# Emieeel/auto_oo

Measured on AMD Instinct MI355X. Metric: OO-VQE energy+grad evals/sec (formaldimine CAS(4e,3o)/cc-pVDZ); 2e-transform fp64 TFLOP/s vs roofline, higher is better.
Workload: dtype f64; 1 GPU; configs[1] shape: N=43 AOs, n_occ=6, CAS(4e,3o), UCCD n_theta=4, n_kappa=327; one step = one batched call evaluating energy + full gradient of all 256 geometries of the rank (256 synthetic geometries in the job, geometry g on rank g mod n_gpus); value = evaluations/s; in-order calls on one stream; geometries_per_rank=256, batched_calls=1332, calls=in order, parallelism=geometry-sharded x1, one all_gather at the end, dist_world_size=1, devices_visible=1, device_of_rank0=0

## Files before the change

auto_oo_amd/csrc/api.hip:

```cpp
#include "common.h"
#include <stdarg.h>
#include <map>
#include <mutex>
#include <tuple>
#include <utility>
#include <vector>

static thread_local char g_err[512] = "";

void oovqe_set_error(const char* fmt, ...)
{
    va_list ap;
    va_start(ap, fmt);
    vsnprintf(g_err, sizeof(g_err), fmt, ap);
    va_end(ap);
}

extern "C" int oovqe_version(void) { return 100; }

extern "C" const char* oovqe_last_error(void) { return g_err; }

extern "C" int oovqe_device_count(void)
{
    int n = 0;
    hipError_t e = hipGetDeviceCount(&n);
    if (e != hipSuccess) {
        oovqe_set_error("hipGetDeviceCount: %s", hipGetErrorString(e));
        return -1;
    }
    return n;
}

int oovqe_ensure_dynamic_lds(const void* kernel, size_t bytes)
{
    static std::mutex mu;
    static std::map<std::pair<const void*, int>, size_t> done;
    int dev = 0;
    if (hipGetDevice(&dev) != hipSuccess) dev = 0;
    std::lock_guard<std::mutex> lock(mu);
    size_t& have = done[std::make_pair(kernel, dev)];
    if (bytes <= have) return 0;
    hipError_t e = hipFuncSetAttribute(kernel, hipFuncAttributeMaxDynamicSharedMemorySize, (int)bytes);
    if (e != hipSuccess) {
        oovqe_set_error("hipFuncSetAttribute(MaxDynamicSharedMemorySize = %zu): %s", bytes, hipGetErrorString(e));
        return OOVQE_ERR_HIP;
    }
    have = bytes;
    return 0;
}

int oovqe_blocks_per_cu(const void* kernel, int threads, size_t lds_bytes)
{
    static std::mutex mu;
    static std::map<std::tuple<const void*, int, int, size_t>, int> known;
    int dev = 0;
    if (hipGetDevice(&dev) != hipSuccess) dev = 0;
    std::lock_guard<std::mutex> lock(mu);
    int& occ = known[std::make_tuple(kernel, dev, threads, lds_bytes)];
    if (occ > 0) return occ;
    int nb = 0;
    OOVQE_CHECK_HIP(hipOccupancyMaxActiveBlocksPerMultiprocessor(&nb, kernel, threads, lds_bytes), "oovqe_blocks_per_cu");
    return occ = nb < 1 ? 1 : nb;
}

int oovqe_cu_count()
{
    static int n_cu[16];
    static std::mutex mu;
    int dev = 0;
    if (hipGetDevice(&dev) != hipSuccess || dev < 0 || dev >= 16) return 256;
    std::lock_guard<std::mutex> lock(mu);
    if (!n_cu[dev]) {
        hipDeviceProp_t prop;
        n_cu[dev] = hipGetDeviceProperties(&prop, dev) == hipSuccess && prop.multiProcessorCount > 0 ? prop.multiProcessorCount : 256;
    }
    return n_cu[dev];
}

static int g_opts[OOVQE_OPT_COUNT] = {0};
static const char* const g_opt_names[OOVQE_OPT_COUNT] = {
    "gm_two_per_cu", "gm_one_per_cu", "fused_chunks", "tri_plain_w", "cas_unfused",
    "sym_no_rs", "sym_mirror", "sym_simple", "sym_two_step", "no_ride", "k1_no_pair", "k1_force_wide", "gm_plain_grid",
    "newton_one_wg", "sector_unfused", "hess_vk_pass", "hess_own_stage1", "panel_rows",
    "k1_force_nt", "newton_no_chol", "sector_lambda_w", "sector_rdm_r3", "panel_no_w",
    "stage1_free_run", "one_stream", "tail_split"};
static_assert(sizeof(g_opt_names) / sizeof(g_opt_names[0]) == OOVQE_OPT_COUNT, "option name table out of step with oovqe_option_t");

int oovqe_opt(int id) { return (id >= 0 && id < OOVQE_OPT_COUNT) ? g_opts[id] : 0; }

static char g_stage1[160] = "";
void oovqe_note_stage1(const char* fmt, ...)
{
    va_list ap;
    va_start(ap, fmt);
    vsnprintf(g_stage1, sizeof(g_stage1), fmt, ap);
    va_end(ap);
}
extern "C" const char* oovqe_last_stage1_kernel(void) { return g_stage1; }

extern "C" int oovqe_debug_set_option(const char* name, int value)
{
    for (int i = 0; name && i < OOVQE_OPT_COUNT; ++i)
        if (strcmp(name, g_opt_names[i]) == 0) { g_opts[i] = value; return 0; }
    oovqe_set_error("oovqe_debug_set_option: unknown option '%s'", name ? name : "(null)");
    return OOVQE_ERR_ARG;
}

extern "C" int oovqe_debug_get_option(const char* name)
{
    for (int i = 0; name && i < OOVQE_OPT_COUNT; ++i)
        if (strcmp(name, g_opt_names[i]) == 0) return g_opts[i];
    return -1;
}

namespace {
struct Internals {
    hipEvent_t ev[64] = {};
    hipStream_t st[1] = {nullptr};
    unsigned next = 0;
    bool tried = false, streams_tried = false;
};
Internals g_int[16];
std::mutex g_int_mu;

Internals* internals()
{
    int dev = 0;
    if (hipGetDevice(&dev) != hipSuccess || dev < 0 || dev >= 16) return nullptr;
    Internals& I = g_int[dev];
    if (!I.tried) {
        I.tried = true;
        for (int i = 0; i < 64; ++i)
            if (hipEventCreateWithFlags(&I.ev[i], hipEventDisableTiming) != hipSuccess) I.ev[i] = nullptr;
    }
    return &I;
}
}

hipEvent_t oovqe_internal_event()
{
    std::lock_guard<std::mutex> lock(g_int_mu);
    Internals* I = internals();
    return I ? I->ev[I->next++ & 63] : nullptr;
}

hipStream_t oovqe_internal_stream(int k)
{
    if (oovqe_opt(OOVQE_OPT_ONE_STREAM) != 0 || k != 0) return nullptr;
    std::lock_guard<std::mutex> lock(g_int_mu);
    Internals* I = internals();
    if (!I) return nullptr;
    if (!I->streams_tried) {
        I->streams_tried = true;
        if (hipStreamCreateWithFlags(&I->st[0], hipStreamNonBlocking) != hipSuccess) I->st[0] = nullptr;
    }
    return I->st[k];
}

static hipStream_t g_s1_stream[16];
static hipEvent_t g_s1_event[16];
static bool g_s1_seen[16];
static int g_s1_multi[16];

int oovqe_stage1_enter(hipStream_t st)
{
    int dev = 0;
    if (hipGetDevice(&dev) != hipSuccess || dev < 0 || dev >= 16) return 0;
    if (oovqe_opt(OOVQE_OPT_STAGE1_FREE_RUN) != 0) return 0;
// ... 123 lines not shown
```

auto_oo_amd/csrc/cas.hip:

```cpp
#include "plan.h"
#include "circuit_small.h"
#include <type_traits>
#include <stdlib.h>

namespace {

constexpr int HALF_WAVES = 8;
constexpr int TRI_REG_R = 3;
constexpr int tiles_depth(int zt) { return zt == 3 ? 4 : 8; }
constexpr int stream_depth(int zt) { return zt == 3 ? 2 : 3; }
constexpr int AUX_PLAIN = 0, AUX_NT = 2;

constexpr int SYM_FULL = 0, SYM_MIRROR = 1, SYM_PACKED = 2;
__device__ __forceinline__ void tri_decode(long t, int N, int& p, int& q)
{
    const double b = 2.0 * N + 1.0;
    int pp = (int)((b - sqrt(b * b - 8.0 * (double)t)) * 0.5);
    pp = pp < 0 ? 0 : (pp > N - 1 ? N - 1 : pp);
    while (pp > 0 && (long)pp * (2 * N - pp + 1) / 2 > t) --pp;
    while (pp < N - 1 && (long)(pp + 1) * (2 * N - pp) / 2 <= t) ++pp;
    p = pp;
    q = pp + (int)(t - (long)pp * (2 * N - pp + 1) / 2);
}

// ... 2333 lines not shown
        int rr[4], cc[4], kk[4];
#pragma unroll
        for (int u = 0; u < 4; ++u) {
            const long idx = base + u * 512 + tid;
            const bool ok = idx < (long)nrdm * n_kappa;
            const long ii = ok ? idx : 0;
            kk[u] = (int)(ii / n_kappa);
            const int t = (int)(ii - (long)kk[u] * n_kappa);
            rr[u] = kap_row[t];
            cc[u] = kap_col[t];
        }
        double frc[4], fcr[4];
#pragma unroll
        for (int u = 0; u < 4; ++u) {
            const double* F = Fcol + (size_t)kk[u] * M * N;
            const int r = rr[u], c = cc[u];
            frc[u] = F[(size_t)(r < M ? r : 0) * N + c] * (r < M ? 1.0 : 0.0);
            fcr[u] = F[(size_t)(c < M ? c : 0) * N + r] * (c < M ? 1.0 : 0.0);
        }
#pragma unroll
        for (int u = 0; u < 4; ++u) {
            const long idx = base + u * 512 + tid;
            if (idx < (long)nrdm * n_kappa) gvec[idx] = 2.0 * (frc[u] - fcr[u]);
        }
    }
    if (fock)
        for (int idx = tid; idx < N * N; idx += 512) {
            const int m = idx / N;
            fock[idx] = m < M ? Fcol[idx] : 0.0;
        }
    if (gmat)
        for (int idx = tid; idx < N * N; idx += 512) {
            const int m = idx / N, n = idx - m * N;
            const double fmn = m < M ? Fcol[(size_t)m * N + n] : 0.0;
            const double fnm = n < M ? Fcol[(size_t)n * N + m] : 0.0;
            gmat[idx] = 2.0 * (fmn - fnm);
        }
    if (tid < nrdm) {
        const int k = tid;
        double acc = 0.0;
        for (int n = 0; n < M; ++n) acc += Epart[(size_t)k * N + n];
        if (k == 0) {
            double core = nuc;
            for (int n = 0; n < M; ++n) core += Cpart[n];
            c0[0] = core;
            E[0] = core + acc;
        } else if (dE) {
            dE[k - 1] = acc;
        }
    }
}

constexpr int TAIL_THREADS = 512;

__host__ __device__ inline bool tail_needed(int x, int y, int z, int no)
{
    const int lo = y < z ? y : z, hi = y < z ? z : y;
    if (lo >= no) return true;
    if (hi < no) return lo == hi || x == lo || x == hi;
    return x >= no || x == lo;
}
__host__ __device__ inline int tail_pitch(int NC) { return 16 * (((NC + 15) / 16) | 1); }

#ifdef OOVQE_TAIL_PROBE
constexpr int TAIL_PROBE_WGS = 512, TAIL_PROBE_MARKS = 32;
__device__ long long g_tail_probe[TAIL_PROBE_WGS][TAIL_PROBE_MARKS];
#define TAIL_MARK(i)                                                                              \
    do {                                                                                          \
        __syncthreads();                                                                          \
        if (threadIdx.x == 0 && blockIdx.x < TAIL_PROBE_WGS && (i) < TAIL_PROBE_MARKS)            \
            g_tail_probe[blockIdx.x][i] = wall_clock64();                                         \
    } while (0)
#else
#define TAIL_MARK(i) do {} while (0)
#endif

template <int KS>
__global__ __launch_bounds__(TAIL_THREADS, 2)
void cas_tail_kernel(const double* __restrict__ J, const double* __restrict__ C, const double* __restrict__ Wpre,
                     const double* __restrict__ gamma, const double* __restrict__ Gamma, int nrdm, int N, int no,
                     int na, int NC, double nuc, const double* __restrict__ nuc_arr,
                     const int32_t* __restrict__ kap_row, const int32_t* __restrict__ kap_col, int n_kappa,
                     double* __restrict__ c0, double* __restrict__ E, double* __restrict__ gvec,
                     double* __restrict__ dE, double* __restrict__ c1, double* __restrict__ c2, size_t out_stride)
{
    extern __shared__ double lds[];
    constexpr int NW = TAIL_THREADS / 64;
    constexpr int PW = (4 * KS + NW - 1) / NW;
    constexpr int GR = 2, NG = (PW + GR - 1) / GR;
    constexpr int NTN = (4 * KS + 15) / 16;
    const int M = no + na, M2 = M * M, M3 = M2 * M;
    const int na2 = na * na, na3 = na2 * na, na4 = na2 * na2;
    const int ncol = M * (M + 1) / 2, nty = (ncol + 15) / 16;
    const long tri = (long)N * (N + 1) / 2;
    const int by = blockIdx.x;
    const int tid = threadIdx.x, lane = tid & 63;
    const int wave = __builtin_amdgcn_readfirstlane(tid >> 6);
    const int lq = lane >> 4, lr = lane & 15;
    {
        const size_t gi = by;
        J += gi * nty * tri * 16;
        C += gi * (size_t)N * N;
        Wpre += gi * (size_t)N * N;
        gamma += gi * (size_t)nrdm * na2;
        Gamma += gi * (size_t)nrdm * na4;
        c0 += gi * out_stride;
        E += gi * out_stride;
        gvec += gi * out_stride;
        if (dE) dE += gi * out_stride;
        c1 += gi * out_stride;
        c2 += gi * out_stride;
        if (nuc_arr) nuc = nuc_arr[gi];
    }
    const int LDG = tail_pitch(NC), nct = (NC + 15) / 16;
    double* Gc = lds;
    double* Cl = Gc + (size_t)4 * KS * LDG;
    double* hn = Cl + (size_t)N * M;
    double* FIn = hn + (size_t)N * M;
    double* gml = FIn + (size_t)N * M;
    double* Gml = gml + (size_t)nrdm * na2;
    double* Cp = Gml + (size_t)nrdm * na4;
    int* tab = reinterpret_cast<int*>(Cp + N);
    int* wcnt = tab + M3;
    int* krow = wcnt + NW;
    int* kcol = krow + n_kappa;
    double* scr = Cp + N + (M3 + NW + 2 * n_kappa + 1) / 2;
    int* tabp = reinterpret_cast<int*>(scr + (size_t)N * N);

    typedef unsigned v2u __attribute__((ext_vector_type(2)));
    constexpr bool COLQ_REGS = KS < 12;
    int colq[KS];
#pragma unroll
    for (int ks = 0; ks < KS; ++ks) {
        const int q = 4 * ks + lq < N ? 4 * ks + lq : N - 1;
        colq[ks] = ((q * (2 * N - q + 1) / 2 - q) * 16 + lr) * (int)sizeof(double);
    }
    const int lin0 = (lq * 16 + lr) * (int)sizeof(double);
    auto load_group = [&](double (&bf)[GR][KS], int ty, int g) {
#pragma unroll
        for (int r = 0; r < GR; ++r) {
            const int i = g * GR + r;
            if (i >= PW) continue;
            int wv = wave;
#if defined(__HIP_DEVICE_COMPILE__)
            asm volatile("" : "+s"(wv));
#endif
            const int p = wv + NW * i;
            int lqo = lq;
#if defined(__HIP_DEVICE_COMPILE__)
            asm volatile("" : "+v"(lqo));
#endif
            const __amdgpu_buffer_rsrc_t jsrd = __builtin_amdgcn_make_buffer_rsrc(
                const_cast<double*>(J + (size_t)(ty < nty ? ty : 0) * tri * 16), 0,
                p < N && ty < nty ? (int)(tri * 16 * sizeof(double)) : 0, 0x00020000);
            const int colp = p * 16 * (int)sizeof(double);
            const int rowp = (p * (2 * N - p + 1) / 2 - p) * 16 * (int)sizeof(double) + lin0;
#pragma unroll
            for (int ks = 0; ks < KS; ++ks) {
                const int q = 4 * ks + lqo;
                const int cq = COLQ_REGS ? colq[ks] : (q * (2 * N - 1 - q) / 2 * 16 + lr) * (int)sizeof(double);
                const int off = lq < p - 4 * ks ? cq + colp : rowp + ks * 64 * (int)sizeof(double);
                const v2u v = __builtin_amdgcn_raw_buffer_load_b64(jsrd, (unsigned)off, 0, 0);
                bf[r][ks] = __builtin_bit_cast(double, v);
            }
        }
    };
    auto mfma_group = [&](const double (&af)[KS], const double (&bf)[GR][KS], const int (&tj)[4], int g) {
#pragma unroll
        for (int r = 0; r < GR; ++r) {
            const int i = g * GR + r;
            if (i >= PW) continue;
            int wv = wave;
#if defined(__HIP_DEVICE_COMPILE__)
            asm volatile("" : "+s"(wv));
#endif
            const int p = wv + NW * i;
            if (p >= 4 * KS) continue;
            d4 acc = d4{0.0, 0.0, 0.0, 0.0};
            if (p < N) {
#pragma unroll
                for (int ks = 0; ks < KS; ++ks) acc = mfma_f64(af[ks], bf[r][ks], acc);
            }
            double* row = Gc + p * LDG;
#pragma unroll
            for (int j = 0; j < 4; ++j)
                if (tj[j] >= 0) row[tj[j]] = acc[j];
        }
    };
    double bs[2][GR][KS];
    TAIL_MARK(0);
#pragma unroll
    for (int s0 = 0; s0 < 2; ++s0) load_group(bs[s0], s0 / NG, s0 % NG);

    for (int idx = tid; idx < N * M; idx += TAIL_THREADS) {
        const int q = idx / M, x = idx - q * M;
        Cl[idx] = C[(size_t)q * N + x];
    }
    for (int idx = tid; idx < N * N; idx += TAIL_THREADS) scr[idx] = Wpre[idx];
    for (int idx = tid; idx < nrdm * na2; idx += TAIL_THREADS) gml[idx] = gamma[idx];
    for (int idx = tid; idx < nrdm * na4; idx += TAIL_THREADS) Gml[idx] = Gamma[idx];
    for (int idx = tid; idx < n_kappa; idx += TAIL_THREADS) {
        krow[idx] = kap_row[idx];
        kcol[idx] = kap_col[idx];
    }
    for (int idx = tid; idx < 4 * KS * (LDG - NC); idx += TAIL_THREADS) {
        const int p = idx / (LDG - NC);
        Gc[p * LDG + NC + (idx - p * (LDG - NC))] = 0.0;
    }
    TAIL_MARK(1);
    {
        const int total = M * ncol;
        int base = 0;
        for (int i0 = 0; i0 < total; i0 += TAIL_THREADS) {
            const int i = i0 + tid;
            int x = 0, y = 0, z = 0;
            bool need = false;
            if (i < total) {
                x = i / ncol;
                tri_decode(i - x * ncol, M, y, z);
                need = tail_needed(x, y, z, no);
            }
            const unsigned long long mask = __ballot(need);
            const int below = __popcll(mask & ((1ull << lane) - 1ull));
            if (lane == 0) wcnt[wave] = __popcll(mask);
            __syncthreads();
            int pre = base, all = 0;
            for (int w = 0; w < NW; ++w) {
                const int c = wcnt[w];
                if (w < wave) pre += c;
                all += c;
            }
            if (i < total) {
                const int v = need ? pre + below : -1;
                tab[(x * M + y) * M + z] = v;
                tab[(x * M + z) * M + y] = v;
                tabp[i] = v;
            }
            __syncthreads();
            base += all;
        }
    }
    TAIL_MARK(2);
    for (int idx = tid; idx < N * M; idx += TAIL_THREADS) {
        const int n = idx / M, x = idx - n * M;
        double acc = 0.0;
        for (int q = 0; q < N; ++q) acc += scr[(size_t)n * N + q] * Cl[q * M + x];
        hn[idx] = acc;
    }
    __syncthreads();
    TAIL_MARK(3);

    {
        double af[KS];
#pragma unroll
        for (int ks = 0; ks < KS; ++ks) {
            const int q = 4 * ks + lq;
            const double c = Cl[(q < N ? q : N - 1) * M + (lr < M ? lr : 0)];
            af[ks] = (q < N && lr < M) ? c : 0.0;
        }
        auto tail_tile = [&](auto par, int ty) {
            constexpr int P = decltype(par)::value;
            const int yz = 16 * ty + lr;
            int tj[4];
#pragma unroll
            for (int j = 0; j < 4; ++j) {
                const int x = lq + 4 * j;
                tj[j] = (x < M && yz < ncol) ? tabp[x * ncol + yz] : -1;
            }
#pragma unroll
            for (int g = 0; g < NG; ++g) {
                mfma_group(af, bs[(P + g) & 1], tj, g);
                __builtin_amdgcn_sched_barrier(0);
                load_group(bs[(P + g) & 1], ty + (g + 2) / NG, (g + 2) % NG);
                __builtin_amdgcn_sched_barrier(0);
            }
        };
        for (int ty = 0; ty < nty; ty += 2) {
            tail_tile(std::integral_constant<int, 0>{}, ty);
            if (ty + 1 < nty) tail_tile(std::integral_constant<int, NG & 1>{}, ty + 1);
        }
    }

    {
        const __amdgpu_buffer_rsrc_t csrd = __builtin_amdgcn_make_buffer_rsrc(
            const_cast<double*>(C), 0, (int)((size_t)N * N * sizeof(double)), 0x00020000);
        double cfa[NTN][KS];
#pragma unroll
        for (int nt = 0; nt < NTN; ++nt)
#pragma unroll
            for (int ks = 0; ks < KS; ++ks) {
                const int pp = 4 * ks + lq, n = 16 * nt + lr;
                const v2u v = __builtin_amdgcn_raw_buffer_load_b64(
                    csrd, (pp < N && n < N) ? (unsigned)((pp * N + n) * (int)sizeof(double)) : 0x7fffffffu, 0, 0);
                cfa[nt][ks] = __builtin_bit_cast(double, v);
            }
        __syncthreads();
        TAIL_MARK(4);
        const int ntn = (N + 15) / 16;
        for (int ct = wave; ct < nct; ct += NW) {
            double* col = Gc + (16 * ct + lr);
            double tf[KS];
#pragma unroll
            for (int ks = 0; ks < KS; ++ks) tf[ks] = col[(4 * ks + lq) * LDG];
#pragma unroll
            for (int nt = 0; nt < NTN; ++nt) {
                if (nt >= ntn) continue;
                d4 acc = d4{0.0, 0.0, 0.0, 0.0};
#pragma unroll
                for (int ks = 0; ks < KS; ++ks) acc = mfma_f64(cfa[nt][ks], tf[ks], acc);
#pragma unroll
                for (int j = 0; j < 4; ++j) {
                    const int n = 16 * nt + lq + 4 * j;
                    if (n < N) col[n * LDG] = acc[j];
                }
            }
        }
        __syncthreads();
        TAIL_MARK(5);
    }

#define TAIL_G(n, a, b, c) Gc[(n) * LDG + tab[((a) * M + (b)) * M + (c)]]
    for (int idx = tid; idx < N * M; idx += TAIL_THREADS) {
        const int n = idx / M, x = idx - n * M;
        double fi = hn[idx];
        for (int i = 0; i < no; ++i) fi += 2.0 * TAIL_G(n, x, i, i) - TAIL_G(n, i, i, x);
        FIn[idx] = fi;
    }
    TAIL_MARK(6);
    double* Fl = scr;
    double* El = Fl + (size_t)nrdm * M * N;
    double* Ga = El + (size_t)nrdm * N;
    double* Dc = Ga + (size_t)N * na3;
    for (int idx = tid; idx < N * na3; idx += TAIL_THREADS) {
        const int n = idx / na3, r = idx - n * na3;
        const int w = r / na2, x = (r / na) % na, y = r % na;
        Ga[idx] = TAIL_G(n, no + w, no + x, no + y);
    }
    for (int idx = tid; idx < N * no * na2; idx += TAIL_THREADS) {
        const int n = idx / (no * na2), r = idx - n * (no * na2);
        const int m = r / na2, v = (r / na) % na, w = r % na;
        const int V = no + v, W = no + w;
        Dc[idx] = TAIL_G(n, m, V, W) - 0.5 * TAIL_G(n, W, V, m);
    }
    __syncthreads();
    TAIL_MARK(7);
    for (int n = tid; n < N; n += TAIL_THREADS) Cp[n] = n < no ? hn[n * M + n] + FIn[n * M + n] : 0.0;
    for (int idx = tid; idx < na * (na + na3); idx += TAIL_THREADS) {
        const int pl = idx / (na + na3), r0 = idx - pl * (na + na3);
        const int n = no + pl;
        if (r0 < na) {
            c1[pl * na + r0] = FIn[n * M + no + r0];
        } else {
            int t = r0 - na;
            const int i3 = t;
            const int s = t % na; t /= na;
            const int r = t % na; t /= na;
            const int q = t;
            c2[(size_t)pl * na3 + i3] = 0.5 * TAIL_G(n, no + q, no + r, no + s);
        }
    }
    TAIL_MARK(8);
    const int ncore = N * nrdm * no;
    for (int idx = tid; idx < N * nrdm * M; idx += TAIL_THREADS) {
        int n, k, m;
        if (idx < ncore) {
            n = idx / (nrdm * no);
            const int r0 = idx - n * (nrdm * no);
            k = r0 / no;
            m = r0 - k * no;
        } else {
            const int j = idx - ncore;
            n = j / (nrdm * na);
            const int r0 = j - n * (nrdm * na);
            k = r0 / na;
            m = no + r0 - k * na;
        }
        const double* FIv = FIn + (size_t)n * M;
        const double* gam = gml + (size_t)k * na2;
        double val;
        if (m < no) {
            const double* Dm = Dc + ((size_t)n * no + m) * na2;
            double fa = 0.0;
            for (int v = 0; v < na; ++v)
                for (int w = 0; w < na; ++w) fa += gam[v * na + w] * Dm[v * na + w];
            val = 2.0 * ((k == 0 ? FIv[m] : 0.0) + fa);
        } else {
            const int v = m - no;
            const double* Gv = Gml + (size_t)k * na4 + (size_t)v * na3;
            double acc = 0.0;
            for (int w = 0; w < na; ++w) acc += FIv[no + w] * gam[v * na + w];
            for (int w = 0; w < na; ++w)
                for (int x = 0; x < na; ++x)
                    for (int y = 0; y < na; ++y)
                        acc += Gv[(w * na + x) * na + y] * Ga[(size_t)n * na3 + (w * na + x) * na + y];
            val = acc;
        }
        Fl[((size_t)k * M + m) * N + n] = val;
    }
    TAIL_MARK(9);
    for (int idx = tid; idx < N * nrdm; idx += TAIL_THREADS) {
        const int n = idx / nrdm, k = idx - n * nrdm;
        double acc = 0.0;
        if (n >= no && n < M) {
            const int p = n - no;
            const double* FIv = FIn + (size_t)n * M;
            const double* gam = gml + (size_t)k * na2 + (size_t)p * na;
            const double* Gpq = Gml + (size_t)k * na4 + (size_t)p * na3;
            for (int q = 0; q < na; ++q) acc += FIv[no + q] * gam[q];
            for (int q = 0; q < na; ++q)
                for (int r = 0; r < na; ++r)
                    for (int s2 = 0; s2 < na; ++s2)
                        acc += 0.5 * Ga[(size_t)n * na3 + (q * na + r) * na + s2] * Gpq[(q * na + r) * na + s2];
        }
        El[(size_t)k * N + n] = acc;
    }
#undef TAIL_G
    __syncthreads();
    TAIL_MARK(10);

    for (int idx = tid; idx < nrdm * n_kappa; idx += TAIL_THREADS) {
        const int k = idx / n_kappa, t = idx - k * n_kappa;
        const int r = krow[t], c = kcol[t];
        const double* F = Fl + (size_t)k * M * N;
        const double frc = F[(size_t)(r < M ? r : 0) * N + c] * (r < M ? 1.0 : 0.0);
        const double fcr = F[(size_t)(c < M ? c : 0) * N + r] * (c < M ? 1.0 : 0.0);
        gvec[idx] = 2.0 * (frc - fcr);
    }
    if (tid < nrdm) {
        const int k = tid;
        double acc = 0.0;
        for (int n = 0; n < M; ++n) acc += El[(size_t)k * N + n];
        if (k == 0) {
            double core = nuc;
            for (int n = 0; n < M; ++n) core += Cp[n];
            c0[0] = core;
            E[0] = core + acc;
        } else if (dE) {
            dE[k - 1] = acc;
        }
    }
    TAIL_MARK(11);
}

}

#ifdef OOVQE_TAIL_PROBE
extern "C" int oovqe_tail_probe_read(long long* out, int n)
{
    const size_t bytes = sizeof(long long) * (size_t)(n < TAIL_PROBE_WGS * TAIL_PROBE_MARKS ? n : TAIL_PROBE_WGS * TAIL_PROBE_MARKS);
    return hipMemcpyFromSymbol(out, HIP_SYMBOL(g_tail_probe), bytes) == hipSuccess ? 0 : 1;
}
#endif

#define OOVQE_STAGE1_DISPATCH(v, LAUNCH, ...)                                                     \
    switch ((v).kch) {                                                                            \
    case 4: LAUNCH(4, 1, 2, ##__VA_ARGS__); break;                                                \
    case 8: LAUNCH(8, 2, 5, ##__VA_ARGS__); break;                                                \
    case 11: LAUNCH(11, 3, 8, ##__VA_ARGS__); break;                                              \
    default: LAUNCH(12, 3, 10, ##__VA_ARGS__); break;                                             \
    }
#define OOVQE_KS_DISPATCH(v, LAUNCH)                                                              \
    switch ((v).ks) {                                                                             \
    case 4: LAUNCH(4); break;                                                                     \
    case 8: LAUNCH(8); break;                                                                     \
    default: LAUNCH(12); break;                                                                   \
    }

static int stage1_variant(int N, Stage1Variant* v)
{
    static const Stage1Variant rows[] = {{4, 1, 2, 4}, {8, 2, 5, 8}, {11, 3, 8, 12}, {12, 3, 10, 12}};
    for (const Stage1Variant& r : rows)
        if (N >= 1 && (N + 3) / 4 <= r.kch) {
            *v = r;
            return 0;
        }
    oovqe_set_error("cas_eval: no stage-1 kernel variant for N=%d", N);
    return OOVQE_ERR_ARG;
}

static size_t half_lds_bytes(int N, int M)
{
    const int ZT = (M + 15) / 16, nrb = (N + 15) / 16, LDM = 16 * (ZT | 1);
    return (((size_t)nrb * 16 * LDM + 511) / 512) * 512 * sizeof(double);
}
static size_t half_lds_bytes_rs(int N, int M) { return half_lds_bytes(N, M) + (size_t)HALF_WAVES * 16 * 17 * sizeof(double); }

static int stage1_half(int N, int M, int sym, bool rs, bool tiles, Stage1* s)
{
    memset(s, 0, sizeof(*s));
    OOVQE_REQUIRE(N >= 1 && M >= 1 && M <= N, "cas_half_transform: bad N=%d M=%d", N, M);
    const int ZT = (M + 15) / 16, nrb = (N + 15) / 16, ksteps = (N + 3) / 4;
    OOVQE_REQUIRE(ZT <= 3, "cas_half_transform: n_occ+ncas = %d > 48 not supported", M);
    OOVQE_REQUIRE(half_lds_bytes(N, M) <= 160 * 1024, "cas_half_transform: N=%d M=%d needs %zu B of LDS", N, M,
                  half_lds_bytes(N, M));
    s->zt = ZT;
    s->sym = sym;
    if (nrb <= 3) {
        s->kernel = S1_HALF;
// ... 191 lines not shown
    oovqe_profile_mark_stop(st);
    OOVQE_CHECK_LAUNCH("cas_eval/sym_q_contract");
    return 0;
}

static int sym_gm_batched(const double* J, const double* C, double* Gm, int N, int M, int batch,
                          hipStream_t st, const oovqe_circuit_job_t* cj, bool packed)
{
    OOVQE_REQUIRE(M >= 1 && M <= 16 && N >= 1 && N <= 48, "sym_gm: N=%d M=%d", N, M);
    Stage1Variant v;
    if (int rc = stage1_variant(N, &v)) return rc;
    size_t lds_bytes = (size_t)4 * v.ks * (M * 16 + 8) * sizeof(double);
    if (cj && cj->lds_bytes > lds_bytes) lds_bytes = cj->lds_bytes;
    const unsigned nty = (unsigned)(((packed ? M * (M + 1) / 2 : M * M) + 15) / 16);
    oovqe_circuit_job_t job;
    memset(&job, 0, sizeof(job));
    if (cj) job = *cj;
    const unsigned nx = nty + (cj ? 1 : 0);
    const bool xcd_grid = oovqe_xcd_grid(batch, oovqe_opt(OOVQE_OPT_GM_PLAIN_GRID) != 0);
    const dim3 grid = xcd_grid ? dim3(nx * (unsigned)((batch + 7) / 8 * 8)) : dim3(nx, batch);
#define OOVQE_LAUNCH_GM2(KS_, WPE_)                                                               \
    do {                                                                                          \
        if (int rc_ = oovqe_ensure_dynamic_lds((const void*)sym_gm_kernel<KS_, WPE_>, lds_bytes)) return rc_; \
        hipLaunchKernelGGL((sym_gm_kernel<KS_, WPE_>), grid, dim3(SMALL_THREADS), lds_bytes, st,  \
                           J, C, Gm, N, M, packed ? 1 : 0, job, cj ? 1 : 0, batch);               \
    } while (0)
    const bool multi_round = ((long)nx * batch > (long)oovqe_cu_count() || oovqe_opt(OOVQE_OPT_GM_TWO_PER_CU)) &&
                             2 * lds_bytes <= 160 * 1024 && oovqe_opt(OOVQE_OPT_GM_ONE_PER_CU) == 0;
#define OOVQE_LAUNCH_GM(KS_)                                                                      \
    do {                                                                                          \
        if (multi_round) OOVQE_LAUNCH_GM2(KS_, 4);                                                \
        else OOVQE_LAUNCH_GM2(KS_, 2);                                                            \
    } while (0)
    oovqe_profile_mark_start_l(st, LABEL_P_TO_N);
    OOVQE_KS_DISPATCH(v, OOVQE_LAUNCH_GM)
    oovqe_profile_mark_stop(st);
#undef OOVQE_LAUNCH_GM
#undef OOVQE_LAUNCH_GM2
    OOVQE_CHECK_LAUNCH("cas_eval/sym_gm");
    return 0;
}

static int tail_depth(int N, const Stage1Variant& v) { return N >= 41 && N <= 44 ? 11 : v.ks; }
#define OOVQE_TAIL_DISPATCH(ks, LAUNCH)                                                           \
    switch (ks) {                                                                                 \
    case 4: LAUNCH(4); break;                                                                     \
    case 8: LAUNCH(8); break;                                                                     \
    case 11: LAUNCH(11); break;                                                                   \
    default: LAUNCH(12); break;                                                                   \
    }

static size_t tail_lds_bytes(int N, int no, int na, int nrdm, int n_kappa, int* NC)
{
    const int M = no + na, M3 = M * M * M;
    Stage1Variant v;
    if (N > 48 || M > 16 || stage1_variant(N, &v)) return 0;
    int nc = 0;
    for (int x = 0; x < M; ++x)
        for (int y = 0; y < M; ++y)
            for (int z = y; z < M; ++z) nc += tail_needed(x, y, z, no) ? 1 : 0;
    *NC = nc;
    const size_t na2 = (size_t)na * na, na4 = na2 * na2;
    size_t scr = (size_t)N * N + ((size_t)M * (M * (M + 1) / 2) + 1) / 2;
    const size_t gc = (size_t)4 * tail_depth(N, v) * tail_pitch(nc);
    const size_t fe = (size_t)nrdm * M * N + (size_t)nrdm * N +
                      (size_t)N * na * na * na + (size_t)N * no * na2;
    if (fe > scr) scr = fe;
    const size_t doubles = gc + 3 * (size_t)N * M + (size_t)nrdm * (na2 + na4) + N +
                           ((size_t)M3 + TAIL_THREADS / 64 + 2 * (size_t)n_kappa + 1) / 2 + scr;
    const size_t bytes = doubles * sizeof(double);
    return bytes <= 160 * 1024 ? bytes : 0;
}

static int cas_tail_batched(const CasEvalArgs& a, const EvalPlan& p, const double* J, const double* Wpre, hipStream_t st)
{
    Stage1Variant v;
    if (int rc = stage1_variant(a.N, &v)) return rc;
#define OOVQE_LAUNCH_TAIL(KS_)                                                                    \
    do {                                                                                          \
        if (int rc_ = oovqe_ensure_dynamic_lds((const void*)cas_tail_kernel<KS_>, p.tail_lds)) return rc_; \
        hipLaunchKernelGGL((cas_tail_kernel<KS_>), dim3(a.batch), dim3(TAIL_THREADS), p.tail_lds, st, J, a.C, Wpre, \
                           a.gamma, a.Gamma, a.nrdm, a.N, a.n_occ, a.ncas, p.tail_nc, a.nuc, a.nuc_arr, a.kap_row, \
                           a.kap_col, a.n_kappa, a.out.c0, a.out.E, a.out.gvec, a.out.dE, a.out.c1, a.out.c2,       \
                           a.out_stride);                                                         \
    } while (0)
    oovqe_profile_mark_start_l(st, LABEL_P_TO_N);
    OOVQE_TAIL_DISPATCH(tail_depth(a.N, v), OOVQE_LAUNCH_TAIL)
    oovqe_profile_mark_stop(st);
#undef OOVQE_LAUNCH_TAIL
    OOVQE_CHECK_LAUNCH("cas_eval/tail");
    return 0;
}

static bool fused_plan(int N, int M, int batch, int n_cu, long chunks_opt, FusedPlan* fp)
{
    if (M > 16 || N > 48 || N < 1) return false;
    const long m2 = (long)M * M, m3 = m2 * M;
    if (chunks_opt <= 0 && (long)batch * N * N < 48L * n_cu) return false;
    long target = n_cu / batch;
    long nchunk0 = chunks_opt > 0 ? chunks_opt : target / N;
    if (nchunk0 < 1) nchunk0 = 1;
    const long cap = (2L * N * m2 - m3) / (m3 + N);
    if (cap < 1) return false;
    if (nchunk0 > cap) nchunk0 = cap;
    int qc = N, nchunk = 1;
    if (nchunk0 > 1) {
        qc = 4 * (int)((N + 4 * nchunk0 - 1) / (4 * nchunk0));
        nchunk = (N + qc - 1) / qc;
    }
    const int QR = (qc + 3) & ~3, CR = (nchunk - 1) * qc + QR;
    int ldb = (int)((m2 + 15) / 16 * 16);
    if (ldb % 32 == 0) ldb += 16;
    const size_t fixed = ((size_t)CR * 16 + 64 + 8) * sizeof(double);
    const size_t block = (size_t)QR * ldb * sizeof(double);
    const size_t task_stage = (size_t)m3 * sizeof(double);
    const long Tg = (long)nchunk * N;
    long wpg = target < 1 ? 1 : target;
    if (wpg > Tg) wpg = Tg;
    const size_t lds_cap = 160 * 1024;
    if (fixed + 2 * block + task_stage > lds_cap) return false;
    const long max_tasks = (long)((lds_cap - fixed - 2 * block) / task_stage);
    if ((Tg + wpg - 1) / wpg > max_tasks) wpg = (Tg + max_tasks - 1) / max_tasks;
    const long ntask = (Tg + wpg - 1) / wpg;
    long nbuf = (long)((lds_cap - fixed - (size_t)ntask * task_stage) / block);
    if (nbuf > 3) nbuf = 3;
    fp->nchunk = nchunk;
    fp->qc = qc;
    fp->nbuf = (int)nbuf;
    fp->ldb = ldb;
    fp->wpg = (int)wpg;
    fp->lds_bytes = fixed + (size_t)nbuf * block + (size_t)ntask * task_stage;
    return true;
}

static int half_transform_fused_batched(const double* g_ao, const double* C, int N, int M, double* T3,
                                        double* Cdup, const FusedPlan& fp, const Stage1& s, int batch, hipStream_t st)
{
#define OOVQE_LAUNCH_FUSED(KC_, NS_, NPC_)                                                        \
    do {                                                                                          \
        if (int rc_lds = oovqe_ensure_dynamic_lds((const void*)half_transform_fused_kernel<KC_, NS_>, 160 * 1024)) return rc_lds; \
        hipLaunchKernelGGL((half_transform_fused_kernel<KC_, NS_>), dim3(fp.wpg, batch),          \
                           dim3(HALF_WAVES * 64), fp.lds_bytes, st, g_ao, C, T3, Cdup, N, M,      \
                           fp.nchunk, fp.qc, fp.nbuf, fp.ldb);                                    \
    } while (0)
    oovqe_note_stage1("%s", s.name);
    oovqe_profile_mark_start(st);
    OOVQE_STAGE1_DISPATCH(s.v, OOVQE_LAUNCH_FUSED)
    oovqe_profile_mark_stop(st);
#undef OOVQE_LAUNCH_FUSED
    OOVQE_CHECK_LAUNCH("cas_eval/half_transform_fused");
    return 0;
}

static unsigned eri_slab_packed_elems(int N) { return eri_slab_pitch(N); }

extern "C" int64_t oovqe_eri_packed_size(int N)
{
    if (N < 1) return 0;
    if (N > 48) {
        const int64_t nst = (N + 15) / 16;
        return (int64_t)N * (N + 1) / 2 * (nst * (nst + 1) / 2) * 256;
    }
    return (int64_t)N * (N + 1) / 2 * eri_slab_packed_elems(N);
}

extern "C" int oovqe_eri_pack(const double* g_ao, int N, int batch, double* packed, oovqe_stream_t stream)
{
    OOVQE_REQUIRE(g_ao && packed, "eri_pack: null pointer");
// ... 843 lines not shown
```

auto_oo_amd/csrc/common.h:

```cpp
#pragma once
#include <hip/hip_runtime.h>
#include <stdint.h>
#include <stdio.h>
#include <string.h>
#include "../../include/oovqe.h"

typedef double d4 __attribute__((ext_vector_type(4)));
typedef double d2 __attribute__((ext_vector_type(2)));
typedef double d2u __attribute__((ext_vector_type(2), aligned(8)));

#define OOVQE_ERR_ARG   (-1)
#define OOVQE_ERR_HIP   (-2)
#define OOVQE_ERR_SIZE  (-3)

void oovqe_set_error(const char* fmt, ...);
void oovqe_profile_mark_start(hipStream_t st);
void oovqe_profile_mark_start_l(hipStream_t st, int label);
void oovqe_profile_mark_stop(hipStream_t st);

enum oovqe_option_t {
    OOVQE_OPT_GM_TWO_PER_CU = 0,
    OOVQE_OPT_GM_ONE_PER_CU,
    OOVQE_OPT_FUSED_CHUNKS,
    OOVQE_OPT_TRI_PLAIN_W,
    OOVQE_OPT_CAS_UNFUSED,
    OOVQE_OPT_SYM_NO_RS,
    OOVQE_OPT_SYM_MIRROR,
    OOVQE_OPT_SYM_SIMPLE,
    OOVQE_OPT_SYM_TWO_STEP,
    OOVQE_OPT_NO_RIDE,
    OOVQE_OPT_K1_NO_PAIR,
    OOVQE_OPT_K1_FORCE_WIDE,
    OOVQE_OPT_GM_PLAIN_GRID,
    OOVQE_OPT_NEWTON_ONE_WG,
    OOVQE_OPT_SECTOR_UNFUSED,
    OOVQE_OPT_HESS_VK_PASS,
    OOVQE_OPT_HESS_OWN_STAGE1,
    OOVQE_OPT_PANEL_ROWS,
    OOVQE_OPT_K1_FORCE_NT,
    OOVQE_OPT_NEWTON_NO_CHOL,
    OOVQE_OPT_SECTOR_LAMBDA_W,
    OOVQE_OPT_SECTOR_RDM_R3,
    OOVQE_OPT_PANEL_NO_W,
    OOVQE_OPT_STAGE1_FREE_RUN,
    OOVQE_OPT_ONE_STREAM,
    OOVQE_OPT_TAIL_SPLIT,
    OOVQE_OPT_COUNT
};
int oovqe_opt(int id);
int oovqe_ensure_dynamic_lds(const void* kernel, size_t bytes);
int oovqe_blocks_per_cu(const void* kernel, int threads, size_t lds_bytes);
int oovqe_cu_count();
void oovqe_note_stage1(const char* fmt, ...);
hipEvent_t oovqe_internal_event();
hipStream_t oovqe_internal_stream(int k);
int oovqe_stage1_enter(hipStream_t st);
int oovqe_stage1_leave(hipStream_t st);

#define OOVQE_CHECK_LAUNCH(name)                                                          \
    do {                                                                                  \
        hipError_t e__ = hipGetLastError();                                               \
        if (e__ != hipSuccess) {                                                          \
            oovqe_set_error("%s: launch failed: %s", name, hipGetErrorString(e__));       \
            return OOVQE_ERR_HIP;                                                         \
        }                                                                                 \
    } while (0)

#define OOVQE_CHECK_HIP(call, name)                                                        \
    do {                                                                                  \
        hipError_t e__ = (call);                                                          \
        if (e__ != hipSuccess) {                                                          \
            oovqe_set_error("%s: %s", name, hipGetErrorString(e__));                      \
            return OOVQE_ERR_HIP;                                                         \
        }                                                                                 \
    } while (0)

#define OOVQE_REQUIRE(cond, ...)                                                          \
    do {                                                                                  \
        if (!(cond)) {                                                                    \
            oovqe_set_error(__VA_ARGS__);                                                 \
            return OOVQE_ERR_ARG;                                                         \
        }                                                                                 \
    } while (0)

struct oovqe_circuit_job_t {
    const double* theta;
    const oovqe_gate_t* gates;
    double* gamma;
    double* Gamma;
    int n_theta, n_gates, n_qubits, ncas, n_tan, count;
    uint32_t init_index;
    size_t lds_bytes;
};

__device__ __forceinline__ d4 mfma_f64(double a, double b, d4 c) {
    return __builtin_amdgcn_mfma_f64_16x16x4f64(a, b, c, 0, 0, 0);
}


__device__ __forceinline__ long clamp_u32(long rem)
{
    int hi = (int)(rem >> 32);
    const unsigned lo = (unsigned)rem;
    asm("" : "+s"(hi));
    return (long)(hi < 0 ? 0u : (hi != 0 ? 0xFFFFFFFFu : lo));
}
```

Before: 602,200 evals/s.

## Prefetch tail inputs into registers and specialize stage-3 gather on active size

The tail kernel now issues buffer loads for the first slices of W, C, the RDMs and kappa indices into registers up front, overlaps them with the index-table setup, and writes them to LDS afterwards. The stage-3 gather that builds Ga/Dc is templated on the active-orbital count (2 or 3) with a 4-way unrolled batch of loads, and a generic fallback sits behind a new option. The aim is to hide global-load latency and cut integer division cost. The price is higher register pressure from the staging arrays and larger code from the template instantiations.

```diff
diff --git a/auto_oo_amd/csrc/api.hip b/auto_oo_amd/csrc/api.hip
--- a/auto_oo_amd/csrc/api.hip
+++ b/auto_oo_amd/csrc/api.hip
@@ -83,7 +83,7 @@
     "sym_no_rs", "sym_mirror", "sym_simple", "sym_two_step", "no_ride", "k1_no_pair", "k1_force_wide", "gm_plain_grid",
     "newton_one_wg", "sector_unfused", "hess_vk_pass", "hess_own_stage1", "panel_rows",
     "k1_force_nt", "newton_no_chol", "sector_lambda_w", "sector_rdm_r3", "panel_no_w",
-    "stage1_free_run", "one_stream", "tail_split"};
+    "stage1_free_run", "one_stream", "tail_split", "tail_generic"};
 static_assert(sizeof(g_opt_names) / sizeof(g_opt_names[0]) == OOVQE_OPT_COUNT, "option name table out of step with oovqe_option_t");
 
 int oovqe_opt(int id) { return (id >= 0 && id < OOVQE_OPT_COUNT) ? g_opts[id] : 0; }
diff --git a/auto_oo_amd/csrc/cas.hip b/auto_oo_amd/csrc/cas.hip
--- a/auto_oo_amd/csrc/cas.hip
+++ b/auto_oo_amd/csrc/cas.hip
@@ -2439,7 +2439,8 @@
                      int na, int NC, double nuc, const double* __restrict__ nuc_arr,
                      const int32_t* __restrict__ kap_row, const int32_t* __restrict__ kap_col, int n_kappa,
                      double* __restrict__ c0, double* __restrict__ E, double* __restrict__ gvec,
-                     double* __restrict__ dE, double* __restrict__ c1, double* __restrict__ c2, size_t out_stride)
+                     double* __restrict__ dE, double* __restrict__ c1, double* __restrict__ c2, size_t out_stride,
+                     int generic)
 {
     extern __shared__ double lds[];
     constexpr int NW = TAIL_THREADS / 64;
@@ -2447,7 +2448,7 @@
     constexpr int GR = 2, NG = (PW + GR - 1) / GR;
     constexpr int NTN = (4 * KS + 15) / 16;
     const int M = no + na, M2 = M * M, M3 = M2 * M;
-    const int na2 = na * na, na3 = na2 * na, na4 = na2 * na2;
+    const int na2 = na * na, na4 = na2 * na2;
     const int ncol = M * (M + 1) / 2, nty = (ncol + 15) / 16;
     const long tri = (long)N * (N + 1) / 2;
     const int by = blockIdx.x;
@@ -2546,25 +2547,64 @@
     };
     double bs[2][GR][KS];
     TAIL_MARK(0);
-#pragma unroll
-    for (int s0 = 0; s0 < 2; ++s0) load_group(bs[s0], s0 / NG, s0 % NG);
-
-    for (int idx = tid; idx < N * M; idx += TAIL_THREADS) {
+
+    constexpr int SW = 5, SC = 2, SG1 = 1, SG2 = 2, SK = 3;
+    double wst[SW], cst[SC], g1st[SG1], g2st[SG2];
+    int krst[SK], kcst[SK];
+    {
+        constexpr int DB = (int)sizeof(double), IB = (int)sizeof(int32_t);
+        const __amdgpu_buffer_rsrc_t wsrd = __builtin_amdgcn_make_buffer_rsrc(
+            const_cast<double*>(Wpre), 0, N * N * DB, 0x00020000);
+        const __amdgpu_buffer_rsrc_t csrd = __builtin_amdgcn_make_buffer_rsrc(
+            const_cast<double*>(C), 0, N * N * DB, 0x00020000);
+        const __amdgpu_buffer_rsrc_t g1srd = __builtin_amdgcn_make_buffer_rsrc(
+            const_cast<double*>(gamma), 0, nrdm * na2 * DB, 0x00020000);
+        const __amdgpu_buffer_rsrc_t g2srd = __builtin_amdgcn_make_buffer_rsrc(
+            const_cast<double*>(Gamma), 0, nrdm * na4 * DB, 0x00020000);
+        const __amdgpu_buffer_rsrc_t krsrd = __builtin_amdgcn_make_buffer_rsrc(
+            const_cast<int32_t*>(kap_row), 0, n_kappa * IB, 0x00020000);
+        const __amdgpu_buffer_rsrc_t kcsrd = __builtin_amdgcn_make_buffer_rsrc(
+            const_cast<int32_t*>(kap_col), 0, n_kappa * IB, 0x00020000);
+#pragma unroll
+        for (int u = 0; u < SW; ++u)
+            wst[u] = __builtin_bit_cast(double, __builtin_amdgcn_raw_buffer_load_b64(wsrd, (unsigned)((tid + u * TAIL_THREADS) * DB), 0, 0));
+#pragma unroll
+        for (int u = 0; u < SC; ++u) {
+            const int idx = tid + u * TAIL_THREADS;
+            const int q = idx / M, x = idx - q * M;
+            cst[u] = __builtin_bit_cast(double, __builtin_amdgcn_raw_buffer_load_b64(
+                csrd, idx < N * M ? (unsigned)((q * N + x) * DB) : 0x7fffffffu, 0, 0));
+        }
+#pragma unroll
+        for (int u = 0; u < SG1; ++u)
+            g1st[u] = __builtin_bit_cast(double, __builtin_amdgcn_raw_buffer_load_b64(g1srd, (unsigned)((tid + u * TAIL_THREADS) * DB), 0, 0));
+#pragma unroll
+        for (int u = 0; u < SG2; ++u)
+            g2st[u] = __builtin_bit_cast(double, __builtin_amdgcn_raw_buffer_load_b64(g2srd, (unsigned)((tid + u * TAIL_THREADS) * DB), 0, 0));
+#pragma unroll
+        for (int u = 0; u < SK; ++u) {
+            krst[u] = __builtin_amdgcn_raw_buffer_load_b32(krsrd, (unsigned)((tid + u * TAIL_THREADS) * IB), 0, 0);
+            kcst[u] = __builtin_amdgcn_raw_buffer_load_b32(kcsrd, (unsigned)((tid + u * TAIL_THREADS) * IB), 0, 0);
+        }
+    }
+    for (int idx = tid + SC * TAIL_THREADS; idx < N * M; idx += TAIL_THREADS) {
         const int q = idx / M, x = idx - q * M;
         Cl[idx] = C[(size_t)q * N + x];
     }
-    for (int idx = tid; idx < N * N; idx += TAIL_THREADS) scr[idx] = Wpre[idx];
-    for (int idx = tid; idx < nrdm * na2; idx += TAIL_THREADS) gml[idx] = gamma[idx];
-    for (int idx = tid; idx < nrdm * na4; idx += TAIL_THREADS) Gml[idx] = Gamma[idx];
-    for (int idx = tid; idx < n_kappa; idx += TAIL_THREADS) {
+    for (int idx = tid + SW * TAIL_THREADS; idx < N * N; idx += TAIL_THREADS) scr[idx] = Wpre[idx];
+    for (int idx = tid + SG1 * TAIL_THREADS; idx < nrdm * na2; idx += TAIL_THREADS) gml[idx] = gamma[idx];
+    for (int idx = tid + SG2 * TAIL_THREADS; idx < nrdm * na4; idx += TAIL_THREADS) Gml[idx] = Gamma[idx];
+    for (int idx = tid + SK * TAIL_THREADS; idx < n_kappa; idx += TAIL_THREADS) {
         krow[idx] = kap_row[idx];
         kcol[idx] = kap_col[idx];
     }
+#pragma unroll
+    for (int s0 = 0; s0 < 2; ++s0) load_group(bs[s0], s0 / NG, s0 % NG);
+
     for (int idx = tid; idx < 4 * KS * (LDG - NC); idx += TAIL_THREADS) {
         const int p = idx / (LDG - NC);
         Gc[p * LDG + NC + (idx - p * (LDG - NC))] = 0.0;
     }
-    TAIL_MARK(1);
     {
         const int total = M * ncol;
         int base = 0;
@@ -2597,6 +2637,26 @@
             base += all;
         }
     }
+    TAIL_MARK(1);
+#pragma unroll
+    for (int u = 0; u < SW; ++u)
+        if (tid + u * TAIL_THREADS < N * N) scr[tid + u * TAIL_THREADS] = wst[u];
+#pragma unroll
+    for (int u = 0; u < SC; ++u)
+        if (tid + u * TAIL_THREADS < N * M) Cl[tid + u * TAIL_THREADS] = cst[u];
+#pragma unroll
+    for (int u = 0; u < SG1; ++u)
+        if (tid + u * TAIL_THREADS < nrdm * na2) gml[tid + u * TAIL_THREADS] = g1st[u];
+#pragma unroll
+    for (int u = 0; u < SG2; ++u)
+        if (tid + u * TAIL_THREADS < nrdm * na4) Gml[tid + u * TAIL_THREADS] = g2st[u];
+#pragma unroll
+    for (int u = 0; u < SK; ++u)
+        if (tid + u * TAIL_THREADS < n_kappa) {
+            krow[tid + u * TAIL_THREADS] = krst[u];
+            kcol[tid + u * TAIL_THREADS] = kcst[u];
+        }
+    __syncthreads();
     TAIL_MARK(2);
     for (int idx = tid; idx < N * M; idx += TAIL_THREADS) {
         const int n = idx / M, x = idx - n * M;
@@ -2677,6 +2737,12 @@
     }
 
 #define TAIL_G(n, a, b, c) Gc[(n) * LDG + tab[((a) * M + (b)) * M + (c)]]
+    double* Fl = scr;
+    double* El = Fl + (size_t)nrdm * M * N;
+    const int na_given = na;
+    auto stage3 = [&](auto nac) {
+    constexpr int NA = decltype(nac)::value;
+    const int na = NA > 0 ? NA : na_given, na2 = na * na, na3 = na2 * na, na4 = na2 * na2;
     for (int idx = tid; idx < N * M; idx += TAIL_THREADS) {
         const int n = idx / M, x = idx - n * M;
         double fi = hn[idx];
@@ -2684,20 +2750,49 @@
         FIn[idx] = fi;
     }
     TAIL_MARK(6);
-    double* Fl = scr;
-    double* El = Fl + (size_t)nrdm * M * N;
     double* Ga = El + (size_t)nrdm * N;
     double* Dc = Ga + (size_t)N * na3;
-    for (int idx = tid; idx < N * na3; idx += TAIL_THREADS) {
-        const int n = idx / na3, r = idx - n * na3;
-        const int w = r / na2, x = (r / na) % na, y = r % na;
-        Ga[idx] = TAIL_G(n, no + w, no + x, no + y);
-    }
-    for (int idx = tid; idx < N * no * na2; idx += TAIL_THREADS) {
-        const int n = idx / (no * na2), r = idx - n * (no * na2);
-        const int m = r / na2, v = (r / na) % na, w = r % na;
-        const int V = no + v, W = no + w;
-        Dc[idx] = TAIL_G(n, m, V, W) - 0.5 * TAIL_G(n, W, V, m);
+    if constexpr (NA > 0) {
+        constexpr int U = 4;
+        for (int b0 = 0; b0 < N * na3; b0 += U * TAIL_THREADS) {
+            double val[U];
+#pragma unroll
+            for (int u = 0; u < U; ++u) {
+                const int idx = b0 + u * TAIL_THREADS + tid < N * na3 ? b0 + u * TAIL_THREADS + tid : 0;
+                const int n = idx / na3, r = idx - n * na3;
+                const int w = r / na2, x = (r / na) % na, y = r % na;
+                val[u] = TAIL_G(n, no + w, no + x, no + y);
+            }
+#pragma unroll
+            for (int u = 0; u < U; ++u)
+                if (b0 + u * TAIL_THREADS + tid < N * na3) Ga[b0 + u * TAIL_THREADS + tid] = val[u];
+        }
+        for (int b0 = 0; b0 < N * no * na2; b0 += U * TAIL_THREADS) {
+            double val[U];
+#pragma unroll
+            for (int u = 0; u < U; ++u) {
+                const int idx = b0 + u * TAIL_THREADS + tid < N * no * na2 ? b0 + u * TAIL_THREADS + tid : 0;
+                const int n = idx / (no * na2), r = idx - n * (no * na2);
+                const int m = r / na2, v = (r / na) % na, w = r % na;
+                const int V = no + v, W = no + w;
+                val[u] = TAIL_G(n, m, V, W) - 0.5 * TAIL_G(n, W, V, m);
+            }
+#pragma unroll
+            for (int u = 0; u < U; ++u)
+                if (b0 + u * TAIL_THREADS + tid < N * no * na2) Dc[b0 + u * TAIL_THREADS + tid] = val[u];
+        }
+    } else {
+        for (int idx = tid; idx < N * na3; idx += TAIL_THREADS) {
+            const int n = idx / na3, r = idx - n * na3;
+            const int w = r / na2, x = (r / na) % na, y = r % na;
+            Ga[idx] = TAIL_G(n, no + w, no + x, no + y);
+        }
+        for (int idx = tid; idx < N * no * na2; idx += TAIL_THREADS) {
+            const int n = idx / (no * na2), r = idx - n * (no * na2);
+            const int m = r / na2, v = (r / na) % na, w = r % na;
+            const int V = no + v, W = no + w;
+            Dc[idx] = TAIL_G(n, m, V, W) - 0.5 * TAIL_G(n, W, V, m);
+        }
     }
     __syncthreads();
     TAIL_MARK(7);
@@ -2771,6 +2866,11 @@
         }
         El[(size_t)k * N + n] = acc;
     }
+    };
+    const int nac = generic ? 0 : na;
+    if (nac == 3) stage3(std::integral_constant<int, 3>{});
+    else if (nac == 2) stage3(std::integral_constant<int, 2>{});
+    else stage3(std::integral_constant<int, 0>{});
 #undef TAIL_G
     __syncthreads();
     TAIL_MARK(10);
@@ -3128,8 +3228,9 @@
         hipLaunchKernelGGL((cas_tail_kernel<KS_>), dim3(a.batch), dim3(TAIL_THREADS), p.tail_lds, st, J, a.C, Wpre, \
                            a.gamma, a.Gamma, a.nrdm, a.N, a.n_occ, a.ncas, p.tail_nc, a.nuc, a.nuc_arr, a.kap_row, \
                            a.kap_col, a.n_kappa, a.out.c0, a.out.E, a.out.gvec, a.out.dE, a.out.c1, a.out.c2,       \
-                           a.out_stride);                                                         \
+                           a.out_stride, generic);                                                \
     } while (0)
+    const int generic = oovqe_opt(OOVQE_OPT_TAIL_GENERIC) != 0;
     oovqe_profile_mark_start_l(st, LABEL_P_TO_N);
     OOVQE_TAIL_DISPATCH(tail_depth(a.N, v), OOVQE_LAUNCH_TAIL)
     oovqe_profile_mark_stop(st);
diff --git a/auto_oo_amd/csrc/common.h b/auto_oo_amd/csrc/common.h
--- a/auto_oo_amd/csrc/common.h
+++ b/auto_oo_amd/csrc/common.h
@@ -45,6 +45,7 @@
     OOVQE_OPT_STAGE1_FREE_RUN,
     OOVQE_OPT_ONE_STREAM,
     OOVQE_OPT_TAIL_SPLIT,
+    OOVQE_OPT_TAIL_GENERIC,
     OOVQE_OPT_COUNT
 };
 int oovqe_opt(int id);
```

Measured after the change: 608,200 evals/s (median of 6 runs). 1.01x the previous value.
